# 3SAILab/two_stage_object_detection

Measured on AMD Instinct MI355X. Metric: images/sec Faster R-CNN ResNet-50 @800x1333, higher is better.
Workload: dtype f32 storage/accumulate; conv products as bf16x3 (3 exact bf16 pieces per operand, 6 bf16 MFMAs per product) in 0 of 43 conv layers, as fp16x2 (2 fp16 pieces of 2^e x per operand, 3 fp16 MFMAs per product; e follows the tensor's abs-max per forward: range words) in 43, f32 MFMA in the rest; 1 GPU; Full Faster R-CNN resnet50 inference forward, batch=1 per GPU, 3x800x1333, 80+1 classes, 3000->300 proposals; global_batch=1, parallelism=dp1, hip_graph=True, autotuned_tiles=True, steps_in_flight=4, tiles_tuned_on=this rank

## Files before the change

### include/tsod.h

```cpp
#ifndef TSOD_H
#define TSOD_H

#include <stddef.h>
#include <stdint.h>

#ifdef __cplusplus
extern "C" {
#endif

#define TSOD_VERSION 242

typedef void *tsod_stream_t;

typedef enum tsod_status {
    TSOD_OK = 0,
    TSOD_ERR_INVALID_ARG = -1,
    TSOD_ERR_UNSUPPORTED = -2,
    TSOD_ERR_ALIGNMENT = -3,
    TSOD_ERR_WORKSPACE = -4,
    TSOD_ERR_LAUNCH = -5
} tsod_status;

const char *tsod_status_str(int status);
int tsod_version(void);
// ... 1 lines not shown

enum { TSOD_ACT_NONE = 0, TSOD_ACT_PRELU = 1, TSOD_ACT_RELU6 = 2, TSOD_ACT_RELU = 3 };
enum { TSOD_TILE_AUTO = 0, TSOD_TILE_128x128 = 1, TSOD_TILE_128x64 = 2, TSOD_TILE_64x64 = 3, TSOD_TILE_64x128 = 4,
       TSOD_TILE_128x128_W8 = 5, TSOD_TILE_128x64_W8 = 6, TSOD_TILE_256x128_W8 = 7, TSOD_TILE_64x64_S1 = 8,
       TSOD_TILE_128x64_W8_S1 = 9, TSOD_TILE_64x64_S1_K64 = 10, TSOD_TILE_128x64_W8_S1_K64 = 11,
       TSOD_TILE_64x64_W1_S1 = 12, TSOD_TILE_128x64_W2_S1 = 13, TSOD_TILE_128x64_S1 = 14, TSOD_TILE_64x128_S1 = 15,
       TSOD_TILE_128x128_S1 = 16,
       TSOD_TILE_D128x128 = 17, TSOD_TILE_D64x128 = 18, TSOD_TILE_D256x128 = 19,
       TSOD_TILE_D64x128_S2 = 20 ,
       TSOD_TILE_D128x256 = 21 ,
       TSOD_TILE_D128x128_K32 = 22 ,
       TSOD_TILE_D192x128 = 23 ,
       TSOD_TILE_D64x128_K64 = 24 ,
       TSOD_TILE_COUNT = 25 };
enum { TSOD_PREC_F32 = 0, TSOD_PREC_BF16X3 = 1, TSOD_PREC_FP16X2 = 2 };
#define TSOD_MAX_SEGMENTS 16

typedef struct tsod_conv2d_desc {
    int32_t N, H, W;
    int32_t in_pitch;
    int32_t n_seg;
    int32_t seg_off[TSOD_MAX_SEGMENTS];
    int32_t seg_len[TSOD_MAX_SEGMENTS];
    int32_t Cout;
    int32_t out_pitch;
    int32_t out_off;
    int32_t KH, KW;
    int32_t stride;
    int32_t pad_h, pad_w;
    int32_t OH, OW;
// ... 17 lines not shown
int tsod_amax_reset(uint32_t *words, int32_t n_tensors, tsod_stream_t stream);
int tsod_absmax_f32(const float *x, int64_t n, uint32_t *amax_out, tsod_stream_t stream);

int tsod_host_mapped_pointer(void *host, void **device);
int tsod_word_publish_i32(const int32_t *src_device, int32_t *dst_mapped, tsod_stream_t stream);

int tsod_pack_conv_weight_f32(const float *w_oihw, int32_t Cout, int32_t Cin_src, int32_t KH, int32_t KW_src,
                              int32_t Cin, int32_t KW, float *w_packed, tsod_stream_t stream);

size_t tsod_conv_weight_bf16x3_bytes(int32_t Cout, int32_t K);
int tsod_pack_conv_weight_bf16x3(const float *w_packed , int32_t Cout, int32_t K, void *w_bf16x3,
                                 tsod_stream_t stream);
size_t tsod_conv_weight_fp16x2_bytes(int32_t Cout, int32_t K);
int tsod_pack_conv_weight_fp16x2(const float *w_packed , int32_t Cout, int32_t K, int32_t w_scale_exp,
                                 void *w_fp16x2, tsod_stream_t stream);

size_t tsod_conv2d_workspace_bytes(const tsod_conv2d_desc *d);
int tsod_conv2d_resolve(const tsod_conv2d_desc *d, int32_t *tile, int32_t *split_k);

int tsod_conv2d_f32(const tsod_conv2d_desc *d, const float *in, const float *w_packed,
                    const float *scale , const float *shift ,
                    const float *residual , float *out,
                    void *workspace, size_t workspace_bytes, tsod_stream_t stream);

int tsod_conv2d_dual_f32(const tsod_conv2d_desc *d, const float *in, const float *in2, const float *w_packed,
                         const float *scale, const float *shift, const float *residual, float *out,
                         void *workspace, size_t workspace_bytes, tsod_stream_t stream);

typedef struct tsod_bottleneck_desc {
    int32_t N, H, W;
// ... 404 lines not shown
```

### two_stage_object_detection_amd/_ffi.py

```python
from __future__ import annotations

import ctypes
import os
from ctypes import POINTER, Structure, byref, c_char_p, c_double, c_float, c_int, c_int32, c_int64, c_size_t, c_void_p
from typing import NamedTuple

import torch

_PKG_DIR = os.path.dirname(os.path.abspath(__file__))
LIB_PATH = os.environ.get("TSOD_LIB") or os.path.join(_PKG_DIR, "libtsod.so")

TSOD_MAX_SEGMENTS = 16
AMAX_WORDS, AMAX_STRIDE = 64, 64
AMAX_BYTES = AMAX_WORDS * AMAX_STRIDE
ACT_NONE, ACT_PRELU, ACT_RELU6, ACT_RELU = 0, 1, 2, 3
PREC_F32, PREC_BF16X3, PREC_FP16X2 = 0, 1, 2
PREC_NAMES = {0: "f32", 1: "bf16x3", 2: "fp16x2"}
TILE_AUTO, TILE_128x128, TILE_128x64, TILE_64x64, TILE_64x128 = 0, 1, 2, 3, 4


class Tile(NamedTuple):
    name: str
    rows: int
    precisions: tuple
# ... 27 lines not shown
    22: Tile("d128x128k32",    128, _SPLIT, dma=True),
    23: Tile("d192x128",       192, _FP16X2, dma=True),
    24: Tile("d64x128k64",     64,  _FP16X2, dma=True),
}


def tile_ids(precision: int) -> tuple:
    return tuple(t for t, row in TILES.items() if precision in row.precisions)


TILE_NAMES = {TILE_AUTO: "auto", **{t: row.name for t, row in TILES.items()}}
TILE_IDS = tile_ids(PREC_F32)
DMA_TILE_IDS = tuple(t for t, row in TILES.items() if row.dma)
BF16X3_TILE_IDS = tile_ids(PREC_BF16X3)
FP16X2_TILE_IDS = tile_ids(PREC_FP16X2)

class TsodError(RuntimeError):
    pass


class ConvDesc(Structure):
    _fields_ = [
        ("N", c_int32), ("H", c_int32), ("W", c_int32),
        ("in_pitch", c_int32), ("n_seg", c_int32),
        ("seg_off", c_int32 * TSOD_MAX_SEGMENTS), ("seg_len", c_int32 * TSOD_MAX_SEGMENTS),
        ("Cout", c_int32), ("out_pitch", c_int32), ("out_off", c_int32),
        ("KH", c_int32), ("KW", c_int32), ("stride", c_int32), ("pad_h", c_int32), ("pad_w", c_int32),
        ("OH", c_int32), ("OW", c_int32), ("act", c_int32), ("slope", c_float),
        ("res_pitch", c_int32), ("res_off", c_int32), ("tile", c_int32), ("split_k", c_int32), ("precision", c_int32),
        ("c2", c_int32), ("in2_pitch", c_int32), ("in2_off", c_int32), ("stride2", c_int32), ("H2", c_int32), ("W2", c_int32),
# ... 46 lines not shown


class GradNormResult(Structure):
    _fields_ = [("sum_sq", c_double), ("norm", c_float), ("coef", c_float)]


_SIGNATURES = {
    "tsod_status_str": (c_char_p, [c_int]),
    "tsod_version": (c_int, []),
    "tsod_device_cu_count": (c_int, []),
    "tsod_pack_conv_weight_f32": (c_int, [c_void_p, c_int32, c_int32, c_int32, c_int32, c_int32, c_int32, c_void_p, c_void_p]),
    "tsod_conv_weight_bf16x3_bytes": (c_size_t, [c_int32, c_int32]),
    "tsod_pack_conv_weight_bf16x3": (c_int, [c_void_p, c_int32, c_int32, c_void_p, c_void_p]),
    "tsod_conv_weight_fp16x2_bytes": (c_size_t, [c_int32, c_int32]),
    "tsod_pack_conv_weight_fp16x2": (c_int, [c_void_p, c_int32, c_int32, c_int32, c_void_p, c_void_p]),
    "tsod_conv2d_workspace_bytes": (c_size_t, [POINTER(ConvDesc)]),
    "tsod_conv2d_resolve": (c_int, [POINTER(ConvDesc), POINTER(c_int32), POINTER(c_int32)]),
    "tsod_conv2d_f32": (c_int, [POINTER(ConvDesc), c_void_p, c_void_p, c_void_p, c_void_p, c_void_p, c_void_p,
                                c_void_p, c_size_t, c_void_p]),
    "tsod_conv2d_dual_f32": (c_int, [POINTER(ConvDesc), c_void_p, c_void_p, c_void_p, c_void_p, c_void_p, c_void_p, c_void_p,
                                     c_void_p, c_size_t, c_void_p]),
    "tsod_bottleneck_wstream_bytes": (c_size_t, [c_int32, c_int32]),
    "tsod_bottleneck_proj_wstream_bytes": (c_size_t, [c_int32, c_int32]),
    "tsod_bottleneck_fp16x2": (c_int, [POINTER(BottleneckDesc), c_void_p, c_void_p, c_void_p, c_void_p, c_void_p]),
    "tsod_stem_wfrag_bytes": (c_size_t, []),
    "tsod_stem_fp16x2": (c_int, [POINTER(StemDesc), c_void_p, c_void_p, c_void_p, c_void_p, c_void_p]),
    "tsod_linear_f32": (c_int, [c_void_p, c_int32, c_int32, c_int32, c_void_p, c_void_p, c_int32, c_void_p, c_int32,
                                c_void_p, c_size_t, c_void_p]),
    "tsod_linear_workspace_bytes": (c_size_t, [c_int32, c_int32, c_int32]),
    "tsod_maxpool3x3s2_f32": (c_int, [c_void_p, c_int32, c_int32, c_int32, c_int32, c_int32, c_void_p, c_int32, c_void_p]),
# ... 295 lines not shown
```

### two_stage_object_detection_amd/csrc/conv_igemm_f32.hip

```cpp
#include "tsod_internal.h"
#include <array>
#include <limits.h>
#include <stdlib.h>

namespace {

typedef float f32x16 __attribute__((ext_vector_type(16)));
typedef __bf16 bf16x8 __attribute__((ext_vector_type(8)));
typedef _Float16 f16x8 __attribute__((ext_vector_type(8)));

constexpr int kPatchLD = 36;
constexpr int kChanTab = 512;

struct ConvParams {
    const float *in, *w, *scale, *shift, *res;
    float *out, *partial;
    int *tickets;
    unsigned part_bytes;
    int N, H, W, in_pitch;
    int n_seg, seg_off[TSOD_MAX_SEGMENTS], seg_end[TSOD_MAX_SEGMENTS];
    int Cin, Cout, out_pitch, out_off;
    int KH, KW, stride, pad_h, pad_w, OH, OW;
    int act;
    float slope;
// ... 1511 lines not shown
int validate(const tsod_conv2d_desc *d) {
    TSOD_REQUIRE(d != nullptr, TSOD_ERR_INVALID_ARG);
    TSOD_REQUIRE(d->N > 0 && d->H > 0 && d->W > 0 && d->Cout > 0 && d->KH > 0 && d->KW > 0, TSOD_ERR_INVALID_ARG);
    TSOD_REQUIRE(d->stride > 0 && d->pad_h >= 0 && d->pad_w >= 0 && d->OH > 0 && d->OW > 0, TSOD_ERR_INVALID_ARG);
    TSOD_REQUIRE(d->n_seg >= 1 && d->n_seg <= TSOD_MAX_SEGMENTS, TSOD_ERR_INVALID_ARG);
    TSOD_REQUIRE((d->in_pitch & 3) == 0 && d->in_pitch > 0, TSOD_ERR_ALIGNMENT);
    for (int s = 0; s < d->n_seg; ++s) {
        TSOD_REQUIRE(d->seg_len[s] > 0 && d->seg_off[s] >= 0, TSOD_ERR_INVALID_ARG);
        TSOD_REQUIRE((d->seg_len[s] & 3) == 0 && (d->seg_off[s] & 3) == 0, TSOD_ERR_ALIGNMENT);
        TSOD_REQUIRE(d->seg_off[s] + d->seg_len[s] <= d->in_pitch, TSOD_ERR_INVALID_ARG);
    }
    TSOD_REQUIRE(d->out_off >= 0 && d->out_pitch >= d->out_off + d->Cout, TSOD_ERR_INVALID_ARG);
    TSOD_REQUIRE((d->OH - 1) * d->stride - d->pad_h < d->H && (d->OW - 1) * d->stride - d->pad_w < d->W,
                 TSOD_ERR_INVALID_ARG);
    TSOD_REQUIRE(d->act >= TSOD_ACT_NONE && d->act <= TSOD_ACT_RELU, TSOD_ERR_INVALID_ARG);
    TSOD_REQUIRE(d->tile >= 0 && d->tile < TSOD_TILE_COUNT && d->split_k >= -2 && d->split_k <= 64, TSOD_ERR_INVALID_ARG);
    TSOD_REQUIRE(d->precision == TSOD_PREC_F32 || d->precision == TSOD_PREC_BF16X3 || d->precision == TSOD_PREC_FP16X2, TSOD_ERR_INVALID_ARG);
    TSOD_REQUIRE(d->tile == TSOD_TILE_AUTO || kTiles[d->tile].launch[d->precision], TSOD_ERR_UNSUPPORTED);
    if (d->precision == TSOD_PREC_FP16X2)
        TSOD_REQUIRE(d->a_scale_exp >= -24 && d->a_scale_exp <= 24 && d->w_scale_exp >= -40 && d->w_scale_exp <= 40, TSOD_ERR_INVALID_ARG);
    const int64_t M = (int64_t)d->N * d->OH * d->OW;
    TSOD_REQUIRE(M < (int64_t)INT_MAX, TSOD_ERR_UNSUPPORTED);
    if (d->c2 != 0) {
        TSOD_REQUIRE(d->c2 > 0 && (d->c2 & 3) == 0 && d->stride2 > 0 && d->H2 > 0 && d->W2 > 0, TSOD_ERR_INVALID_ARG);
        TSOD_REQUIRE((d->in2_pitch & 3) == 0 && (d->in2_off & 3) == 0, TSOD_ERR_ALIGNMENT);
        TSOD_REQUIRE(d->in2_off >= 0 && d->in2_off + d->c2 <= d->in2_pitch, TSOD_ERR_INVALID_ARG);
        TSOD_REQUIRE((d->OH - 1) * d->stride2 < d->H2 && (d->OW - 1) * d->stride2 < d->W2, TSOD_ERR_INVALID_ARG);
        TSOD_REQUIRE(d->n_seg == 1 && (d->KH * d->KW * d->seg_len[0]) % 32 == 0 && d->seg_len[0] % 32 == 0, TSOD_ERR_UNSUPPORTED);
    }
    return TSOD_OK;
}
// ... 152 lines not shown
    }
    return best;
}

uint64_t weight_image_bytes(int prec, int Cout, int K) {
    const uint64_t groups = (uint64_t)Cout * ((K + 7) / 8);
    return prec == TSOD_PREC_BF16X3 ? groups * 48 : prec == TSOD_PREC_FP16X2 ? groups * 32 : (uint64_t)Cout * K * sizeof(float);
}

}

extern "C" int tsod_conv2d_resolve(const tsod_conv2d_desc *d, int32_t *tile, int32_t *split_k) {
    const int rc = validate(d);
    if (rc != TSOD_OK) return rc;
    TSOD_REQUIRE(tile && split_k, TSOD_ERR_INVALID_ARG);
    const Sched s = resolve(d);
    TSOD_REQUIRE(s.cost < 1e299, TSOD_ERR_UNSUPPORTED);
    *tile = s.tile;
    *split_k = s.sk_q > 0 ? -2 : (s.rem_tiles == 0 ? 1 : (s.dp_tiles == 0 ? s.split : -1));
    return TSOD_OK;
}

extern "C" size_t tsod_conv2d_workspace_bytes(const tsod_conv2d_desc *d) {
    if (validate(d) != TSOD_OK) return 0;
    const Sched s = resolve(d);
    return s.cost < 1e299 ? s.ws_bytes : 0;
}

extern "C" int tsod_conv2d_f32(const tsod_conv2d_desc *d, const float *in, const float *w_packed, const float *scale,
                               const float *shift, const float *residual, float *out, void *workspace,
                               size_t workspace_bytes, tsod_stream_t stream) {
    if (d != nullptr && d->c2 != 0) return TSOD_ERR_INVALID_ARG;
    return tsod_conv2d_dual_f32(d, in, nullptr, w_packed, scale, shift, residual, out, workspace, workspace_bytes, stream);
}

extern "C" int tsod_conv2d_dual_f32(const tsod_conv2d_desc *d, const float *in, const float *in2, const float *w_packed,
                                    const float *scale, const float *shift, const float *residual, float *out,
                                    void *workspace, size_t workspace_bytes, tsod_stream_t stream) {
    const int rc = validate(d);
    if (rc != TSOD_OK) return rc;
    TSOD_REQUIRE(in && w_packed && out, TSOD_ERR_INVALID_ARG);
    TSOD_REQUIRE((d->c2 > 0) == (in2 != nullptr) && (!in2 || tsod_aligned16(in2)), TSOD_ERR_INVALID_ARG);
    TSOD_REQUIRE(tsod_aligned16(in) && tsod_aligned16(w_packed), TSOD_ERR_ALIGNMENT);
    if (residual) TSOD_REQUIRE(d->res_off >= 0 && d->res_pitch >= d->res_off + d->Cout, TSOD_ERR_INVALID_ARG);

    ConvParams p;
    p.in = in; p.w = w_packed; p.scale = scale; p.shift = shift; p.res = residual; p.out = out;
    p.N = d->N; p.H = d->H; p.W = d->W; p.in_pitch = d->in_pitch;
    p.n_seg = d->n_seg;
    int cum = 0;
    for (int s = 0; s < TSOD_MAX_SEGMENTS; ++s) {
        p.seg_off[s] = s < d->n_seg ? d->seg_off[s] : 0;
        if (s < d->n_seg) cum += d->seg_len[s];
        p.seg_end[s] = cum;
    }
    p.Cin = cum; p.Cout = d->Cout; p.out_pitch = d->out_pitch; p.out_off = d->out_off;
    p.KH = d->KH; p.KW = d->KW; p.stride = d->stride; p.pad_h = d->pad_h; p.pad_w = d->pad_w;
    p.OH = d->OH; p.OW = d->OW; p.act = d->act; p.slope = d->slope;
    p.res_pitch = d->res_pitch; p.res_off = d->res_off;
// ... 142 lines not shown
```

### two_stage_object_detection_amd/engine.py

```python
from __future__ import annotations

import math
from collections import OrderedDict
from ctypes import byref, c_int32
from typing import Callable, Sequence

import torch

from . import _ffi
from ._ffi import (ACT_NONE, ACT_PRELU, ACT_RELU, ACT_RELU6, TILE_NAMES, ConvDesc, TsodError, check, lib,
                   make_conv_desc, ptr, stream_ptr)


def fold_bn(bn: torch.nn.BatchNorm2d):
    var = bn.running_var.detach().double().cpu()
    mean = bn.running_mean.detach().double().cpu()
    gamma = bn.weight.detach().double().cpu() if bn.affine else torch.ones_like(var)
    beta = bn.bias.detach().double().cpu() if bn.affine else torch.zeros_like(var)
    scale = gamma / torch.sqrt(var + bn.eps)
    shift = beta - mean * scale
    return scale.float(), shift.float()


class PackedConv:
# ... 140 lines not shown
def fp16x2_activation_exp(absmax: float, headroom_bits: int = 4) -> int:
    if absmax == 0.0 or not math.isfinite(absmax):
        return 8
    return max(-24, min(8, int(math.floor(math.log2(65504.0 / (absmax * (1 << headroom_bits)))))))


def weights_fp16x2(pc):
    hit = getattr(pc, "w2", None)
    if hit is None:
        from . import hip_ops
        e = hip_ops.fp16x2_weight_scale_exp(pc.w)
        hit = pc.w2 = (_publish(hip_ops.pack_conv_weight_fp16x2(pc.w, e)), e)
    return hit


def prelu_slope(m: torch.nn.PReLU) -> float:
    if m.weight.numel() != 1:
        raise TsodError("only single-parameter nn.PReLU is supported (what the reference uses)")
    return float(m.weight.detach().cpu().item())


class BufferPool:

    def __init__(self, device):
        self.device = device
        self._free: dict[int, list[torch.Tensor]] = {}
        self.total_bytes = 0
        self.on_alloc = None

    def alloc(self, shape: Sequence[int], dtype=torch.float32) -> torch.Tensor:
# ... 21 lines not shown
        if out and out[-1][0] + out[-1][1] == off:
            out[-1] = (out[-1][0], out[-1][1] + ln)
        else:
            out.append((off, ln))
    return out


class ConvStep:
    __slots__ = ("desc", "args", "name", "flops", "ws_bytes", "pc", "fn", "plan", "x", "x2")
    W_ARG, WS_ARG = 3, 8

    def choose(self, tile: int, split_k: int, precision: int):
        d = self.desc
        d.tile, d.split_k, d.precision = int(tile), int(split_k), int(precision)
        if precision == _ffi.PREC_FP16X2:
            w2, e = weights_fp16x2(self.pc)
            d.a_scale_exp, d.w_scale_exp = int(self.plan.a_exps.get(self.name, FP16X2_A_SCALE_EXP)), int(e)
            d.range_flag = ptr(self.plan.range_flag)
            self.args[self.W_ARG] = ptr(w2)
        else:
            self.args[self.W_ARG] = ptr(weights_bf16x3(self.pc)) if precision == _ffi.PREC_BF16X3 else ptr(self.pc.w)

    def args_on(self, ws: torch.Tensor) -> list:
        a = list(self.args)
        a[self.WS_ARG], a[self.WS_ARG + 1] = ptr(ws), ws.numel()
        return a


class Plan:
    def __init__(self, device, packed: dict | None = None, *, range_flag=None, a_exps: dict | None = None, slot: int = 0,
                 on_calibrated=None, precision: int = 0):
# ... 293 lines not shown
            d = st.desc
            K = d.KH * d.KW * sum(d.seg_len[i] for i in range(d.n_seg)) + max(0, int(d.c2))
            ksteps = (K + 31) // 32
            M = d.N * d.OH * d.OW
            self._refresh_amax_for(st)
            cands = []
            for prec in (precisions if precisions is not None else (int(d.precision),)):
                for tile in _ffi.tile_ids(prec):
                    for split in (splits or (1, -1, -2, 2, 3, 4, 6, 8, 12, 16, 24, 32)):
                        if split > 1 and ksteps // split < 2:
                            continue
                        st.choose(tile, split, prec)
                        if lib().tsod_conv2d_workspace_bytes(byref(d)) > big.numel():
                            continue
                        cands.append((tile, split, prec))
            def time_candidate(tile, split, prec, n_reps):
                st.choose(tile, split, prec)
                args = st.args_on(big)
                s = stream_ptr()
                conv_fn = st.fn
                rc = conv_fn(*args, s)
                if rc != 0:
                    return None
                e0, e1 = torch.cuda.Event(enable_timing=True), torch.cuda.Event(enable_timing=True)
                if concurrent == 1:
                    e0.record()
                    for _ in range(n_reps):
                        rc |= conv_fn(*args, s)
                    e1.record()
                else:
# ... 36 lines not shown
                raise TsodError(f"autotune: no runnable (tile, split) candidate for {st.name}")
            def beyond_l2(tile, split, prec):
                st.choose(tile, split, prec)
                slabs = max(0, int(lib().tsod_conv2d_workspace_bytes(byref(d))) - (256 << 10))
                wbytes = d.Cout * K * (6 if prec == _ffi.PREC_BF16X3 else 4)
                tiles_m = -(-M // _ffi.TILES[tile].rows)
                return 2 * slabs + wbytes * (tiles_m if split == -2 else 8)
            close = [c for c in second_look if c[0] <= best[0] * 1.02]
            if len(close) > 1:
                best = min(close, key=lambda c: (beyond_l2(c[1], c[2], c[3]), c[0]))
            st.choose(best[1], best[2], best[3])
            n_short = max(1, int(in_sequence), int(keep_shortlist))
            if n_short > 1:
                short, per = [], {}
                for c in timed:
                    if per.get((c[1], c[3]), 0) < 2:
                        short.append(c)
                        per[(c[1], c[3])] = per.get((c[1], c[3]), 0) + 1
                    if len(short) >= n_short:
                        break
                for pr in sorted({c[3] for c in timed}):
                    if all(c[3] != pr for c in short):
                        short.append(next(c for c in timed if c[3] == pr))
            else:
                short = list(timed[:1])
            shortlist.append([(tile, split, prec) for _, tile, split, prec in short])
            by = {}
            for t_, tile, split, prec in timed:
                by.setdefault(prec, (tile, split))
            best_by_prec.append(by)
            results.append((st.name, best[0], best[1], best[2], st.flops, best[3]))
            if verbose:
                print(f"  {st.name:34s} {TILE_NAMES[best[1]]:8s} split {best[2]:3d} {_ffi.PREC_NAMES[best[3]]:6s} {best[0] * 1e3:8.1f} us "
# ... 410 lines not shown
```

### two_stage_object_detection_amd/hip_ops.py

```python
from __future__ import annotations

import contextlib
import ctypes
import math
import threading
from ctypes import byref, c_int32

import torch
from torch.autograd.function import once_differentiable

from . import _ffi
from ._ffi import ACT_NONE, TsodError, check, lib, make_conv_desc, ptr, require_cuda, stream_ptr


class _Arena:

    def __init__(self, zero: bool = False):
        self._buf = {}
        self._retired = {}
        self._zero = zero

    def _key(self, device):
        owner = getattr(_OWNER_TLS, "owner", None)
        if owner is not None:
# ... 81 lines not shown
    return out


def fp16x2_weight_scale_exp(w_packed: torch.Tensor) -> int:
    m = float(w_packed.abs().max())
    return 0 if m == 0.0 or not math.isfinite(m) else max(-40, min(40, int(math.floor(math.log2(16384.0 / m)))))


def pack_conv_weight_fp16x2(w_packed: torch.Tensor, w_scale_exp: int) -> torch.Tensor:
    require_cuda(w_packed, "pack_conv_weight_fp16x2")
    w_packed = w_packed.contiguous()
    cout = w_packed.shape[0]
    K = w_packed.numel() // cout
    out = torch.empty(lib().tsod_conv_weight_fp16x2_bytes(cout, K), dtype=torch.uint8, device=w_packed.device)
    check(lib().tsod_pack_conv_weight_fp16x2(ptr(w_packed), cout, K, int(w_scale_exp), ptr(out), stream_ptr()), "pack_conv_weight_fp16x2")
    return out


_W3_CACHE: dict = {}


def _w3_for(w_packed: torch.Tensor) -> torch.Tensor:
    if w_packed.is_inference():
        return pack_conv_weight_bf16x3(w_packed)
    key = (w_packed.data_ptr(), tuple(w_packed.shape), w_packed._version)
    hit = _W3_CACHE.get(key)
    if hit is None:
        if len(_W3_CACHE) >= 64:
            _W3_CACHE.clear()
        base = w_packed._base if w_packed._base is not None else w_packed
# ... 18 lines not shown
        Cout, KH, KW, Cin = w_packed.shape
    segs = [(0, Cin)] if segs is None else segs
    assert sum(s[1] for s in segs) == Cin, "segments must add up to the packed Cin"
    OH = (H + 2 * pad - KH) // stride + 1
    OW = (W + 2 * pad - (KW if kw_logical is None else kw_logical)) // stride + 1
    if out is None:
        out = torch.empty((N, OH, OW, Cout), dtype=torch.float32, device=x.device)
    assert out.is_contiguous() and out.shape[:3] == (N, OH, OW)
    d = make_conv_desc(N=N, H=H, W=W, in_pitch=P, segs=segs, Cout=Cout, out_pitch=out.shape[3], out_off=out_off,
                       KH=KH, KW=KW, stride=stride, pad_h=pad, pad_w=pad, OH=OH, OW=OW, act=act, slope=slope,
                       res_pitch=0 if residual is None else residual.shape[-1], res_off=0, tile=tile, split_k=split_k,
                       precision=precision, src2=src2)
    if precision == _ffi.PREC_FP16X2:
        if w2 is None:
            w_scale_exp = fp16x2_weight_scale_exp(w_packed)
            w2 = pack_conv_weight_fp16x2(w_packed, w_scale_exp)
        d.a_scale_exp, d.w_scale_exp = int(a_scale_exp), int(w_scale_exp)
        d.range_flag = ptr(range_flag)
        d.amax_in, d.amax_in2 = _word_ptr(amax_in), _word_ptr(amax_in2)
    d.amax_out = _word_ptr(amax_out)
    ws_bytes = lib().tsod_conv2d_workspace_bytes(byref(d))
    ws = CONV_ARENA.get(x.device, ws_bytes) if ws_bytes else None
    w_arg = (w3 if w3 is not None else _w3_for(w_packed)) if precision == _ffi.PREC_BF16X3 else (w2 if precision == _ffi.PREC_FP16X2 else w_packed)
    check(lib().tsod_conv2d_dual_f32(byref(d), ptr(x), ptr(x2), ptr(w_arg), ptr(scale), ptr(shift), ptr(residual), ptr(out),
                                     ptr(ws), ws_bytes, stream_ptr()), "conv2d")
    return out


def pack_bottleneck_wstream(w1: torch.Tensor, w2: torch.Tensor, w3: torch.Tensor, projection: bool = False):
    dev = w1.device
    cin, cout = w1.shape[1], w3.shape[0]
# ... 1485 lines not shown
```

### two_stage_object_detection_amd/models/hardnet_grads.py

```python
from __future__ import annotations

import torch
from torch.autograd.function import once_differentiable

from .. import _ffi, hip_ops
from ..engine import bn_fold_grads, bnt_copy


def _conv33_weight(d, C):
    return d[:, :, :C].reshape(9, C).t().reshape(C, 1, 3, 3)


def pw_copy(rec):
    rc, y = rec["rc"], rec["y"]
    return dict(index=rec["index"], off=rec["off"], cout=rec["cout"], segs=rec["segs"], seg_real=rec["seg_real"],
                slices=rec["slices"], w=rc.w.view(rc.cout, -1).clone(), scale=rc.scale.clone(), bn=rec["bn"],
                y=None if y is None else y[..., rec["y_off"]:rec["y_off"] + rc.cout].clone(), bnt=bnt_copy(rec.get("bnt")))


def dw_copy(rec):
    return dict(rec, dw=tuple(t.clone() if isinstance(t, torch.Tensor) else t for t in rec["dw"]),
                x=None if rec["x"] is None else (rec["x"][0].clone(), rec["x"][1]), dw_bnt=bnt_copy(rec.get("dw_bnt")))


# ... 131 lines not shown
    if getattr(old, "w3", None) is not None:
        old.w3.copy_(hip_ops.pack_conv_weight_bf16x3(old.w))
    if getattr(old, "w2", None) is not None:
        img, e = old.w2
        top = float(old.w.abs().max()) * 2.0 ** e
        if not (2.0 ** 12 <= top < 2.0 ** 15):
            e = hip_ops.fp16x2_weight_scale_exp(old.w)
            for plan in owner._plans.values():
                for st in plan.conv_steps:
                    if getattr(st.pc, "pack", st.pc) is old and int(st.desc.precision) == _ffi.PREC_FP16X2:
                        st.desc.w_scale_exp = int(e)
                        plan.graph = None
            owner._bump_version()
        img.copy_(hip_ops.pack_conv_weight_fp16x2(old.w, e))
        old.w2 = (img, e)


def copy_pack(owner, old, new):
    for o, t in zip(old, new):
        if isinstance(o, torch.Tensor):
            o.copy_(t)


def refresh_packs(owner):
    start = owner.__dict__.get("_watch_from")
    if start is None:
        return
    seen = owner.__dict__.setdefault("_pack_versions", {})
    stale = {}
    for u in owner._units():
# ... 11 lines not shown
```

Measured before the change: 1172 images/s.

## Add activation-resident fp16x2 expand kernel for 1x1 convs with autotuned split codes

Adds a dedicated kernel for stride-1 1x1 fp16x2 convolutions. It loads a full row panel of the input (K up to 512) into LDS once as hi/lo fp16 pieces, then streams pre-swizzled weights for several 64-channel output slices over that resident panel, with fused scale, shift, residual, activation and amax epilogue. New negative split_k codes select the panel size and slice grouping, and these codes are added as candidates to the tile autotuner. The aim is to stop re-reading and re-splitting the activations for every output tile. The cost is a second packed weight copy per eligible layer and more autotune candidates.

```diff
diff --git a/include/tsod.h b/include/tsod.h
--- a/include/tsod.h
+++ b/include/tsod.h
@@ -39,6 +39,8 @@
        TSOD_TILE_D64x128_K64 = 24 ,
        TSOD_TILE_COUNT = 25 };
 enum { TSOD_PREC_F32 = 0, TSOD_PREC_BF16X3 = 1, TSOD_PREC_FP16X2 = 2 };
+#define TSOD_SPLIT_EXPAND (-3)
+#define TSOD_SPLIT_EXPAND_FORCED (-4)
 #define TSOD_MAX_SEGMENTS 16
 
 typedef struct tsod_conv2d_desc {
@@ -86,6 +88,9 @@
 size_t tsod_conv_weight_fp16x2_bytes(int32_t Cout, int32_t K);
 int tsod_pack_conv_weight_fp16x2(const float *w_packed , int32_t Cout, int32_t K, int32_t w_scale_exp,
                                  void *w_fp16x2, tsod_stream_t stream);
+size_t tsod_conv_weight_expand_fp16x2_bytes(int32_t Cout, int32_t K);
+int tsod_pack_conv_weight_expand_fp16x2(const float *w_packed , int32_t Cout, int32_t K, int32_t w_scale_exp,
+                                        void *wstream, tsod_stream_t stream);
 
 size_t tsod_conv2d_workspace_bytes(const tsod_conv2d_desc *d);
 int tsod_conv2d_resolve(const tsod_conv2d_desc *d, int32_t *tile, int32_t *split_k);
diff --git a/two_stage_object_detection_amd/_ffi.py b/two_stage_object_detection_amd/_ffi.py
--- a/two_stage_object_detection_amd/_ffi.py
+++ b/two_stage_object_detection_amd/_ffi.py
@@ -65,6 +65,18 @@
 DMA_TILE_IDS = tuple(t for t, row in TILES.items() if row.dma)
 BF16X3_TILE_IDS = tile_ids(PREC_BF16X3)
 FP16X2_TILE_IDS = tile_ids(PREC_FP16X2)
+TILE_64x128_S1 = 15
+SPLIT_EXPAND, SPLIT_EXPAND_FORCED = -3, -4
+EXPAND_SPLITS = tuple(range(SPLIT_EXPAND, SPLIT_EXPAND_FORCED - 10, -1))
+
+
+def expand_split(rows: int, groups: int) -> int:
+    return SPLIT_EXPAND_FORCED - ((rows // 128) + 2 * (int(groups).bit_length() - 1))
+
+
+def is_expand_split(split_k: int) -> bool:
+    return SPLIT_EXPAND_FORCED - 9 <= int(split_k) <= SPLIT_EXPAND
+
 
 class TsodError(RuntimeError):
     pass
@@ -141,6 +153,8 @@
     "tsod_pack_conv_weight_bf16x3": (c_int, [c_void_p, c_int32, c_int32, c_void_p, c_void_p]),
     "tsod_conv_weight_fp16x2_bytes": (c_size_t, [c_int32, c_int32]),
     "tsod_pack_conv_weight_fp16x2": (c_int, [c_void_p, c_int32, c_int32, c_int32, c_void_p, c_void_p]),
+    "tsod_conv_weight_expand_fp16x2_bytes": (c_size_t, [c_int32, c_int32]),
+    "tsod_pack_conv_weight_expand_fp16x2": (c_int, [c_void_p, c_int32, c_int32, c_int32, c_void_p, c_void_p]),
     "tsod_conv2d_workspace_bytes": (c_size_t, [POINTER(ConvDesc)]),
     "tsod_conv2d_resolve": (c_int, [POINTER(ConvDesc), POINTER(c_int32), POINTER(c_int32)]),
     "tsod_conv2d_f32": (c_int, [POINTER(ConvDesc), c_void_p, c_void_p, c_void_p, c_void_p, c_void_p, c_void_p,
diff --git a/two_stage_object_detection_amd/csrc/conv_expand.h b/two_stage_object_detection_amd/csrc/conv_expand.h
--- /dev/null
+++ b/two_stage_object_detection_amd/csrc/conv_expand.h
@@ -0,0 +1,68 @@
+#pragma once
+#include <stdint.h>
+#include "../../include/tsod.h"
+
+#if defined(__HIPCC__)
+#define TSOD_EXPAND_HD __host__ __device__
+#else
+#define TSOD_EXPAND_HD
+#endif
+
+constexpr int kExpandForcedLast = TSOD_SPLIT_EXPAND_FORCED - 9;
+static inline bool tsod_expand_split(int split_k) { return split_k <= TSOD_SPLIT_EXPAND && split_k >= kExpandForcedLast; }
+
+constexpr int kExpandPatchBytes = 32 * 144;
+constexpr int kExpandLdsMax = 160 * 1024;
+
+TSOD_EXPAND_HD static inline int tsod_expand_pitch(int K) { return 2 * K + 16; }
+TSOD_EXPAND_HD static inline int tsod_expand_lds_bytes(int R, int K) { return 2 * R * tsod_expand_pitch(K) + 4 * kExpandPatchBytes + 64; }
+
+TSOD_EXPAND_HD static inline int tsod_expand_pi(int j) { return 16 * ((j >> 2) & 1) + 4 * (j >> 3) + (j & 3); }
+TSOD_EXPAND_HD static inline int tsod_expand_pi_inv(int r) { return (((r >> 2) & 3) << 3) | ((r >> 4) << 2) | (r & 3); }
+TSOD_EXPAND_HD static inline size_t tsod_expand_stream_offset(int K, int n, int g) {
+    const int q = n >> 6, cb = (n >> 5) & 1, j = tsod_expand_pi_inv(n & 31);
+    const int s = g >> 2, c = (g >> 1) & 1, hh = g & 1;
+    return ((size_t)(q * (K / 32) + s) * 2 + cb) * 4096 + (size_t)(32 * hh + j) * 64 + c * 32;
+}
+
+static inline bool tsod_expand_shape_ok(const tsod_conv2d_desc *d) {
+    if (d->precision != TSOD_PREC_FP16X2 || d->KH != 1 || d->KW != 1 || d->stride != 1 || d->pad_h != 0 || d->pad_w != 0) return false;
+    if (d->n_seg != 1 || d->c2 > 0 || d->OH != d->H || d->OW != d->W) return false;
+    const int K = d->seg_len[0];
+    if (K % 32 != 0 || K < 64 || K > 512 || d->Cout <= 0 || d->Cout % 64 != 0) return false;
+    if ((d->seg_off[0] | d->out_pitch | d->out_off | d->res_pitch | d->res_off) & 3) return false;
+    return true;
+}
+
+struct tsod_expand_pick_t {
+    int R, G, groups;
+};
+
+static inline bool tsod_expand_pick(int64_t M, int K, int Cout, int cus, int split_k, tsod_expand_pick_t *out) {
+    const int slices = Cout / 64;
+    if (split_k != TSOD_SPLIT_EXPAND) {
+        const int code = TSOD_SPLIT_EXPAND_FORCED - split_k, R = 64 << (code & 1);
+        int groups = 1 << (code >> 1);
+        if (tsod_expand_lds_bytes(R, K) > kExpandLdsMax) return false;
+        if (groups > slices) groups = slices;
+        out->R = R; out->G = (slices + groups - 1) / groups; out->groups = (slices + out->G - 1) / out->G;
+        return true;
+    }
+    double best = 1e300;
+    for (int R = 64; R <= 128; R += 64) {
+        if (tsod_expand_lds_bytes(R, K) > kExpandLdsMax) continue;
+        const int64_t panels = (M + R - 1) / R;
+        for (int G = slices; G >= 1; --G) {
+            const int groups = (slices + G - 1) / G;
+            if ((slices + groups - 1) / groups != G) continue;
+            const int64_t per_cu = (panels * groups + cus - 1) / cus;
+            const double work = (double)R * K / 256.0 + (double)G * (R / 64) * (3.0 * K / 16.0 + 10.0);
+            const double cost = (double)per_cu * work;
+            if (cost < best) { best = cost; out->R = R; out->G = G; out->groups = groups; }
+        }
+    }
+    return best < 1e299;
+}
+
+int tsod_conv_expand_launch(const tsod_conv2d_desc *d, const float *in, const void *wstream, const float *scale, const float *shift,
+                            const float *residual, float *out, tsod_stream_t stream);
diff --git a/two_stage_object_detection_amd/csrc/conv_expand.hip b/two_stage_object_detection_amd/csrc/conv_expand.hip
--- /dev/null
+++ b/two_stage_object_detection_amd/csrc/conv_expand.hip
@@ -0,0 +1,333 @@
+#include "tsod_internal.h"
+#include "conv_expand.h"
+#include <limits.h>
+
+namespace {
+
+typedef float f32x16 __attribute__((ext_vector_type(16)));
+typedef unsigned int u32x4 __attribute__((ext_vector_type(4)));
+
+constexpr unsigned kOOB = 0xFFFFFFF0u;
+constexpr int W_STEP = 8192;
+constexpr int P_PITCH = 144, P_BYTES = kExpandPatchBytes;
+
+struct ExpandParams {
+    const float *in, *res, *scale, *shift;
+    float *out;
+    const unsigned char *wstream;
+    int M, K, slices, G, groups;
+    unsigned in_row, in_off, out_row, out_off, res_row, res_off;
+    unsigned in_bytes, out_bytes, res_bytes;
+    float neg_slope, act_hi;
+    float a_scale, acc_scale;
+    int w_scale_exp;
+    const unsigned *amax_in;
+    unsigned *amax_out;
+    int *range_flag;
+};
+
+__device__ __forceinline__ float4 bload4(__amdgpu_buffer_rsrc_t r, unsigned off) {
+    const u32x4 v = __builtin_amdgcn_raw_buffer_load_b128(r, off, 0, 0);
+    return make_float4(__uint_as_float(v.x), __uint_as_float(v.y), __uint_as_float(v.z), __uint_as_float(v.w));
+}
+__device__ __forceinline__ float act(float v, float neg_slope, float hi) { return fminf(fmaxf(v, 0.f) + neg_slope * fminf(v, 0.f), hi); }
+
+struct WFrag { u32x4 h[2], l[2]; };
+struct AFrag { u32x4 h, l; };
+
+template <int R, int RING>
+__global__ void __launch_bounds__(256, 2) conv_expand_kernel(const ExpandParams p) {
+    constexpr int NB = R / 64;
+    constexpr int SLOTS = RING ? RING : 3, AHEAD = SLOTS - 1;
+    extern __shared__ __align__(16) unsigned char lds[];
+    const int tid = threadIdx.x, lane = tid & 63, wave = tid >> 6;
+    const int j = lane & 31, hh = lane >> 5;
+    const int cb = wave & 1, pb0 = wave >> 1;
+    const int pitch = tsod_expand_pitch(p.K), plane = R * pitch, KS = p.K >> 5;
+    unsigned char *patch = lds + 2 * plane + wave * P_BYTES;
+    float *scr = reinterpret_cast<float *>(lds + 2 * plane + 4 * P_BYTES);
+
+    const int nwg = (int)gridDim.x, per = nwg >> 3, r8 = nwg & 7, xcd = (int)blockIdx.x & 7;
+    const int item = (xcd < r8 ? xcd * (per + 1) : r8 * (per + 1) + (xcd - r8) * per) + ((int)blockIdx.x >> 3);
+    const int panel = item / p.groups, grp = item - panel * p.groups;
+    const int m0 = panel * R, q_begin = grp * p.G, q_end = min(q_begin + p.G, p.slices);
+    const __amdgpu_buffer_rsrc_t rs_x = __builtin_amdgcn_make_buffer_rsrc((void *)p.in, (short)0, (int)p.in_bytes, 0x00020000);
+    const __amdgpu_buffer_rsrc_t rs_o = __builtin_amdgcn_make_buffer_rsrc((void *)p.out, (short)0, (int)p.out_bytes, 0x00020000);
+    const __amdgpu_buffer_rsrc_t rs_r = __builtin_amdgcn_make_buffer_rsrc((void *)(p.res ? p.res : p.out), (short)0, (int)p.res_bytes, 0x00020000);
+
+    float a_scale = p.a_scale, acc_scale = p.acc_scale;
+    if (p.amax_in != nullptr) {
+        const int e = tsod_fp16x2_exp_from_bits(tsod_amax_reduce_bits(p.amax_in[lane * TSOD_AMAX_STRIDE_WORDS]));
+        a_scale = __uint_as_float((unsigned)(127 + e) << 23);
+        acc_scale = __uint_as_float((unsigned)(127 - e - p.w_scale_exp) << 23);
+    }
+    a_scale = __uint_as_float((unsigned)__builtin_amdgcn_readfirstlane((int)__float_as_uint(a_scale)));
+    acc_scale = __uint_as_float((unsigned)__builtin_amdgcn_readfirstlane((int)__float_as_uint(acc_scale)));
+
+    const int t_end = q_end * KS;
+    const u32x4 *wbase = reinterpret_cast<const u32x4 *>(p.wstream + cb * (W_STEP / 2) + lane * 64);
+    auto w_load = [&](int s, WFrag &f) {
+        if (s >= t_end) return;
+        const u32x4 *src = wbase + (size_t)s * (W_STEP / 16);
+        f.h[0] = src[0]; f.l[0] = src[1]; f.h[1] = src[2]; f.l[1] = src[3];
+    };
+    WFrag wf[SLOTS];
+    int t = q_begin * KS;
+#pragma unroll
+    for (int i = 0; i < AHEAD; ++i) w_load(t + i, wf[i]);
+    wf[AHEAD] = wf[0];
+
+    const int upr = p.K >> 2, n_it = (R * upr) >> 8;
+    const int drow = 256 / upr, dq = 256 - drow * upr;
+    int lrow = tid / upr, lq = tid - lrow * upr, srow = lrow, sq = lq;
+    auto advance = [&](int &row, int &q) {
+        row += drow; q += dq;
+        if (q >= upr) { q -= upr; ++row; }
+    };
+    auto x_load = [&](int it, float4 (&x)[4]) {
+#pragma unroll
+        for (int i = 0; i < 4; ++i) {
+            if (it + i >= n_it) break;
+            const int m = m0 + lrow;
+            x[i] = bload4(rs_x, m < p.M ? (unsigned)m * p.in_row + p.in_off + (unsigned)lq * 16u : kOOB);
+            advance(lrow, lq);
+        }
+    };
+    auto x_store = [&](int it, const float4 (&x)[4]) {
+#pragma unroll
+        for (int i = 0; i < 4; ++i) {
+            if (it + i >= n_it) break;
+            unsigned h0, l0, h1, l1;
+            tsod_split2_pair(x[i].x, x[i].y, a_scale, h0, l0);
+            tsod_split2_pair(x[i].z, x[i].w, a_scale, h1, l1);
+            unsigned char *dst = lds + srow * pitch + sq * 8;
+            *reinterpret_cast<uint2 *>(dst) = make_uint2(h0, h1);
+            *reinterpret_cast<uint2 *>(dst + plane) = make_uint2(l0, l1);
+            advance(srow, sq);
+        }
+    };
+    {
+        float4 xa[4], xb[4];
+        x_load(0, xa);
+        for (int it = 0; it < n_it; it += 8) {
+            x_load(it + 4, xb);
+            x_store(it, xa);
+            x_load(it + 8, xa);
+            x_store(it + 4, xb);
+        }
+    }
+
+    const int ep_px = lane >> 3, ep_q = lane & 7;
+    int afa[NB];
+    unsigned opix[NB][4], rpix[NB][4];
+#pragma unroll
+    for (int b = 0; b < NB; ++b) {
+        afa[b] = ((pb0 + 2 * b) * 32 + j) * pitch + hh * 16;
+#pragma unroll
+        for (int i = 0; i < 4; ++i) {
+            const int m = m0 + (pb0 + 2 * b) * 32 + ep_px + 8 * i;
+            const unsigned ch = (unsigned)(cb * 32 + ep_q * 4) * 4u;
+            opix[b][i] = m < p.M ? (unsigned)m * p.out_row + p.out_off + ch : kOOB;
+            rpix[b][i] = m < p.M ? (unsigned)m * p.res_row + p.res_off + ch : kOOB;
+        }
+    }
+    auto res_load = [&](int q, float4 (&r)[NB][4]) {
+        const unsigned chq = (unsigned)(q * 64) * 4u;
+#pragma unroll
+        for (int b = 0; b < NB; ++b)
+#pragma unroll
+            for (int i = 0; i < 4; ++i) r[b][i] = bload4(rs_r, (q < q_end && rpix[b][i] != kOOB) ? rpix[b][i] + chq : kOOB);
+    };
+    auto a_frags = [&](int off, AFrag (&f)[NB]) {
+#pragma unroll
+        for (int b = 0; b < NB; ++b) {
+            f[b].h = *reinterpret_cast<const u32x4 *>(lds + afa[b] + off);
+            f[b].l = *reinterpret_cast<const u32x4 *>(lds + afa[b] + off + plane);
+        }
+    };
+    float4 res_next[NB][4];
+    res_load(q_begin, res_next);
+    __syncthreads();
+
+    float amax = 0.f, chk = 0.f;
+    f32x16 acc[NB];
+    AFrag af[2][NB];
+    for (int q = q_begin; q < q_end; ++q) {
+        float4 res[NB][4];
+#pragma unroll
+        for (int b = 0; b < NB; ++b)
+#pragma unroll
+            for (int i = 0; i < 4; ++i) res[b][i] = res_next[b][i];
+        res_load(q + 1, res_next);
+#pragma unroll
+        for (int b = 0; b < NB; ++b)
+#pragma unroll
+            for (int e = 0; e < 16; ++e) acc[b][e] = 0.f;
+        a_frags(0, af[0]);
+        auto step = [&](int ks, const WFrag &w) {
+            a_frags(ks * 64 + 32, af[1]);
+#pragma unroll
+            for (int b = 0; b < NB; ++b) tsod_mfma3(acc[b], w.h[0], w.l[0], af[0][b].h, af[0][b].l);
+            if (ks + 1 < KS) a_frags(ks * 64 + 64, af[0]);
+#pragma unroll
+            for (int b = 0; b < NB; ++b) tsod_mfma3(acc[b], w.h[1], w.l[1], af[1][b].h, af[1][b].l);
+        };
+        if constexpr (RING == 0) {
+            for (int ks = 0; ks < KS; ++ks, ++t) {
+                w_load(t + 2, wf[2]);
+                step(ks, wf[0]);
+                wf[0] = wf[1];
+                wf[1] = wf[2];
+            }
+        } else {
+            for (int ks0 = 0; ks0 < KS; ks0 += RING) {
+#pragma unroll
+                for (int i = 0; i < RING; ++i, ++t) {
+                    w_load(t + AHEAD, wf[(i + AHEAD) % RING]);
+                    step(ks0 + i, wf[i]);
+                    __builtin_amdgcn_sched_barrier(0);
+                }
+            }
+        }
+        const unsigned chq = (unsigned)(q * 64) * 4u;
+        const int ch = q * 64 + cb * 32 + ep_q * 4;
+        float4 sv = make_float4(acc_scale, acc_scale, acc_scale, acc_scale), bv = make_float4(0.f, 0.f, 0.f, 0.f);
+        if (p.scale != nullptr) {
+            const float4 s4 = *reinterpret_cast<const float4 *>(p.scale + ch);
+            sv = make_float4(s4.x * acc_scale, s4.y * acc_scale, s4.z * acc_scale, s4.w * acc_scale);
+        }
+        if (p.shift != nullptr) bv = *reinterpret_cast<const float4 *>(p.shift + ch);
+#pragma unroll
+        for (int b = 0; b < NB; ++b) {
+#pragma unroll
+            for (int v = 0; v < 4; ++v) {
+                chk = fmaf(acc[b][4 * v], 0.f, fmaf(acc[b][4 * v + 1], 0.f, fmaf(acc[b][4 * v + 2], 0.f, fmaf(acc[b][4 * v + 3], 0.f, chk))));
+                *reinterpret_cast<float4 *>(patch + j * P_PITCH + (16 * hh + 4 * v) * 4) =
+                    make_float4(acc[b][4 * v], acc[b][4 * v + 1], acc[b][4 * v + 2], acc[b][4 * v + 3]);
+            }
+            asm volatile("s_waitcnt lgkmcnt(0)" ::: "memory");
+            float4 tt[4];
+#pragma unroll
+            for (int i = 0; i < 4; ++i) tt[i] = *reinterpret_cast<const float4 *>(patch + (ep_px + 8 * i) * P_PITCH + ep_q * 16);
+            asm volatile("s_waitcnt lgkmcnt(0)" ::: "memory");
+            float m4 = 0.f;
+#pragma unroll
+            for (int i = 0; i < 4; ++i) {
+                const float o0 = act(fmaf(tt[i].x, sv.x, bv.x + res[b][i].x), p.neg_slope, p.act_hi);
+                const float o1 = act(fmaf(tt[i].y, sv.y, bv.y + res[b][i].y), p.neg_slope, p.act_hi);
+                const float o2 = act(fmaf(tt[i].z, sv.z, bv.z + res[b][i].z), p.neg_slope, p.act_hi);
+                const float o3 = act(fmaf(tt[i].w, sv.w, bv.w + res[b][i].w), p.neg_slope, p.act_hi);
+                const float m = fmaxf(fmaxf(fabsf(o0), fabsf(o1)), fmaxf(fabsf(o2), fabsf(o3)));
+                m4 = fmaxf(m4, opix[b][i] != kOOB ? m : 0.f);
+                u32x4 o;
+                o.x = __float_as_uint(o0); o.y = __float_as_uint(o1); o.z = __float_as_uint(o2); o.w = __float_as_uint(o3);
+                __builtin_amdgcn_raw_buffer_store_b128(o, rs_o, opix[b][i] != kOOB ? opix[b][i] + chq : kOOB, 0, 0);
+            }
+            amax = fmaxf(amax, m4);
+        }
+    }
+    if (p.range_flag != nullptr && __any(!(chk == 0.f)) && lane == 0) atomicOr(p.range_flag, 1);
+    if (p.amax_out != nullptr) tsod_amax_commit(p.amax_out, amax, scr, tid, 256);
+}
+
+__global__ void __launch_bounds__(256)
+pack_weight_expand_kernel(const float *__restrict__ w, int Cout, int K, float scale, unsigned char *__restrict__ out) {
+    const int groups = K / 8;
+    const long total = (long)Cout * groups;
+    for (long t = (long)blockIdx.x * blockDim.x + threadIdx.x; t < total; t += (long)gridDim.x * blockDim.x) {
+        const int g = (int)(t % groups), n = (int)(t / groups);
+        u32x4 h, l;
+#pragma unroll
+        for (int e = 0; e < 4; ++e) {
+            const int k = g * 8 + 2 * e;
+            unsigned hv, lv;
+            tsod_split2_pair(w[(long)n * K + k], w[(long)n * K + k + 1], scale, hv, lv);
+            h[e] = hv;
+            l[e] = lv;
+        }
+        u32x4 *o = reinterpret_cast<u32x4 *>(out + tsod_expand_stream_offset(K, n, g));
+        o[0] = h;
+        o[1] = l;
+    }
+}
+
+int expand_cus() {
+    static const int cus = [] {
+        int dev = 0, n = 0;
+        if (hipGetDevice(&dev) == hipSuccess && hipDeviceGetAttribute(&n, hipDeviceAttributeMultiprocessorCount, dev) == hipSuccess && n > 0) return n;
+        (void)hipGetLastError();
+        return 256;
+    }();
+    return cus;
+}
+
+template <int R, int RING>
+bool expand_lds_ready() {
+    static const bool ok = hipFuncSetAttribute(reinterpret_cast<const void *>(conv_expand_kernel<R, RING>),
+                                               hipFuncAttributeMaxDynamicSharedMemorySize, kExpandLdsMax) == hipSuccess;
+    if (!ok) (void)hipGetLastError();
+    return ok;
+}
+
+}
+
+int tsod_conv_expand_launch(const tsod_conv2d_desc *d, const float *in, const void *wstream, const float *scale, const float *shift,
+                            const float *residual, float *out, tsod_stream_t stream) {
+    TSOD_REQUIRE(tsod_expand_shape_ok(d), TSOD_ERR_UNSUPPORTED);
+    TSOD_REQUIRE(tsod_aligned16(in) && tsod_aligned16(wstream) && tsod_aligned16(out) && (!residual || tsod_aligned16(residual)) &&
+                     (!scale || tsod_aligned16(scale)) && (!shift || tsod_aligned16(shift)), TSOD_ERR_ALIGNMENT);
+    TSOD_REQUIRE((reinterpret_cast<uintptr_t>(d->amax_in) & 63u) == 0 && (reinterpret_cast<uintptr_t>(d->amax_out) & 63u) == 0, TSOD_ERR_ALIGNMENT);
+    const int64_t M = (int64_t)d->N * d->H * d->W;
+    const int K = d->seg_len[0];
+    const uint64_t in_bytes = (uint64_t)M * d->in_pitch * 4, out_bytes = (uint64_t)M * d->out_pitch * 4;
+    const uint64_t res_bytes = residual ? (uint64_t)M * d->res_pitch * 4 : 0;
+    TSOD_REQUIRE(M < INT_MAX && in_bytes < 0xFFFFFFF0ull && out_bytes < 0xFFFFFFF0ull && res_bytes < 0xFFFFFFF0ull, TSOD_ERR_UNSUPPORTED);
+    tsod_expand_pick_t pick;
+    TSOD_REQUIRE(tsod_expand_pick(M, K, d->Cout, expand_cus(), d->split_k, &pick), TSOD_ERR_UNSUPPORTED);
+    ExpandParams p;
+    p.in = in; p.res = residual; p.scale = scale; p.shift = shift; p.out = out; p.wstream = static_cast<const unsigned char *>(wstream);
+    p.M = (int)M; p.K = K; p.slices = d->Cout / 64; p.G = pick.G; p.groups = pick.groups;
+    p.in_row = (unsigned)d->in_pitch * 4u; p.in_off = (unsigned)d->seg_off[0] * 4u;
+    p.out_row = (unsigned)d->out_pitch * 4u; p.out_off = (unsigned)d->out_off * 4u;
+    p.res_row = (unsigned)d->res_pitch * 4u; p.res_off = (unsigned)d->res_off * 4u;
+    p.in_bytes = (unsigned)in_bytes; p.out_bytes = (unsigned)out_bytes; p.res_bytes = (unsigned)res_bytes;
+    p.neg_slope = d->act == TSOD_ACT_NONE ? 1.f : (d->act == TSOD_ACT_PRELU ? d->slope : 0.f);
+    p.act_hi = d->act == TSOD_ACT_RELU6 ? 6.f : __builtin_huge_valf();
+    p.a_scale = ldexpf(1.f, d->a_scale_exp); p.acc_scale = ldexpf(1.f, -(d->a_scale_exp + d->w_scale_exp));
+    p.w_scale_exp = d->w_scale_exp;
+    p.amax_in = d->amax_in; p.amax_out = d->amax_out; p.range_flag = d->range_flag;
+    const int64_t grid = (M + pick.R - 1) / pick.R * pick.groups;
+    TSOD_REQUIRE(grid < 0x7FFFFFFF, TSOD_ERR_UNSUPPORTED);
+    const size_t lds = (size_t)tsod_expand_lds_bytes(pick.R, K);
+    const int ring = K % 256 == 0 ? 8 : (K % 128 == 0 ? 4 : 0);
+#define TSOD_EXPAND_LAUNCH(R_, RING_)                                                                                            \
+    do {                                                                                                                         \
+        TSOD_REQUIRE((expand_lds_ready<R_, RING_>()), TSOD_ERR_LAUNCH);                                                          \
+        hipLaunchKernelGGL((conv_expand_kernel<R_, RING_>), dim3((unsigned)grid), dim3(256), lds, tsod_stream(stream), p);       \
+    } while (0)
+    if (pick.R == 64) {
+        if (ring == 8) TSOD_EXPAND_LAUNCH(64, 8); else if (ring == 4) TSOD_EXPAND_LAUNCH(64, 4); else TSOD_EXPAND_LAUNCH(64, 0);
+    } else {
+        if (ring >= 4) TSOD_EXPAND_LAUNCH(128, 4); else TSOD_EXPAND_LAUNCH(128, 0);
+    }
+#undef TSOD_EXPAND_LAUNCH
+    return tsod_launch_status();
+}
+
+extern "C" size_t tsod_conv_weight_expand_fp16x2_bytes(int32_t Cout, int32_t K) {
+    if (Cout <= 0 || K <= 0 || Cout % 64 || K % 32) return 0;
+    return (size_t)(Cout / 64) * (K / 32) * W_STEP;
+}
+
+extern "C" int tsod_pack_conv_weight_expand_fp16x2(const float *w_packed, int32_t Cout, int32_t K, int32_t w_scale_exp, void *wstream,
+                                                   tsod_stream_t stream) {
+    TSOD_REQUIRE(w_packed && wstream, TSOD_ERR_INVALID_ARG);
+    TSOD_REQUIRE(Cout > 0 && K > 0 && w_scale_exp >= -40 && w_scale_exp <= 40, TSOD_ERR_INVALID_ARG);
+    TSOD_REQUIRE(Cout % 64 == 0 && K % 32 == 0, TSOD_ERR_UNSUPPORTED);
+    TSOD_REQUIRE(tsod_aligned16(wstream), TSOD_ERR_ALIGNMENT);
+    const long total = (long)Cout * (K / 8);
+    const int blocks = (int)(tsod_cdiv(total, 256) < 4096 ? tsod_cdiv(total, 256) : 4096);
+    hipLaunchKernelGGL(pack_weight_expand_kernel, dim3(blocks), dim3(256), 0, tsod_stream(stream), w_packed, Cout, K,
+                       ldexpf(1.f, w_scale_exp), static_cast<unsigned char *>(wstream));
+    return tsod_launch_status();
+}
diff --git a/two_stage_object_detection_amd/csrc/conv_igemm_f32.hip b/two_stage_object_detection_amd/csrc/conv_igemm_f32.hip
--- a/two_stage_object_detection_amd/csrc/conv_igemm_f32.hip
+++ b/two_stage_object_detection_amd/csrc/conv_igemm_f32.hip
@@ -2,6 +2,7 @@
 #include <array>
 #include <limits.h>
 #include <stdlib.h>
+#include "conv_expand.h"
 
 namespace {
 
@@ -1549,7 +1550,9 @@
     TSOD_REQUIRE((d->OH - 1) * d->stride - d->pad_h < d->H && (d->OW - 1) * d->stride - d->pad_w < d->W,
                  TSOD_ERR_INVALID_ARG);
     TSOD_REQUIRE(d->act >= TSOD_ACT_NONE && d->act <= TSOD_ACT_RELU, TSOD_ERR_INVALID_ARG);
-    TSOD_REQUIRE(d->tile >= 0 && d->tile < TSOD_TILE_COUNT && d->split_k >= -2 && d->split_k <= 64, TSOD_ERR_INVALID_ARG);
+    TSOD_REQUIRE(d->tile >= 0 && d->tile < TSOD_TILE_COUNT && d->split_k <= 64 &&
+                     (d->split_k >= -2 || (tsod_expand_split(d->split_k) && d->tile == TSOD_TILE_64x128_S1 && d->precision == TSOD_PREC_FP16X2)),
+                 TSOD_ERR_INVALID_ARG);
     TSOD_REQUIRE(d->precision == TSOD_PREC_F32 || d->precision == TSOD_PREC_BF16X3 || d->precision == TSOD_PREC_FP16X2, TSOD_ERR_INVALID_ARG);
     TSOD_REQUIRE(d->tile == TSOD_TILE_AUTO || kTiles[d->tile].launch[d->precision], TSOD_ERR_UNSUPPORTED);
     if (d->precision == TSOD_PREC_FP16X2)
@@ -1732,6 +1735,14 @@
     const int rc = validate(d);
     if (rc != TSOD_OK) return rc;
     TSOD_REQUIRE(tile && split_k, TSOD_ERR_INVALID_ARG);
+    if (tsod_expand_split(d->split_k)) {
+        tsod_expand_pick_t pick;
+        TSOD_REQUIRE(tsod_expand_shape_ok(d) && tsod_expand_pick((int64_t)d->N * d->H * d->W, d->seg_len[0], d->Cout, cu_count(), d->split_k, &pick),
+                     TSOD_ERR_UNSUPPORTED);
+        *tile = d->tile;
+        *split_k = d->split_k;
+        return TSOD_OK;
+    }
     const Sched s = resolve(d);
     TSOD_REQUIRE(s.cost < 1e299, TSOD_ERR_UNSUPPORTED);
     *tile = s.tile;
@@ -1740,7 +1751,7 @@
 }
 
 extern "C" size_t tsod_conv2d_workspace_bytes(const tsod_conv2d_desc *d) {
-    if (validate(d) != TSOD_OK) return 0;
+    if (validate(d) != TSOD_OK || tsod_expand_split(d->split_k)) return 0;
     const Sched s = resolve(d);
     return s.cost < 1e299 ? s.ws_bytes : 0;
 }
@@ -1761,6 +1772,8 @@
     TSOD_REQUIRE((d->c2 > 0) == (in2 != nullptr) && (!in2 || tsod_aligned16(in2)), TSOD_ERR_INVALID_ARG);
     TSOD_REQUIRE(tsod_aligned16(in) && tsod_aligned16(w_packed), TSOD_ERR_ALIGNMENT);
     if (residual) TSOD_REQUIRE(d->res_off >= 0 && d->res_pitch >= d->res_off + d->Cout, TSOD_ERR_INVALID_ARG);
+    if (tsod_expand_split(d->split_k))
+        return tsod_conv_expand_launch(d, in, w_packed, scale, shift, residual, out, stream);
 
     ConvParams p;
     p.in = in; p.w = w_packed; p.scale = scale; p.shift = shift; p.res = residual; p.out = out;
diff --git a/two_stage_object_detection_amd/engine.py b/two_stage_object_detection_amd/engine.py
--- a/two_stage_object_detection_amd/engine.py
+++ b/two_stage_object_detection_amd/engine.py
@@ -178,6 +178,22 @@
     return hit
 
 
+def weights_expand(pc):
+    hit = getattr(pc, "wx", None)
+    if hit is None:
+        from . import hip_ops
+        e = weights_fp16x2(pc)[1]
+        hit = pc.wx = (_publish(hip_ops.pack_conv_weight_expand_fp16x2(pc.w, e)), e)
+    return hit
+
+
+def expand_eligible(d) -> bool:
+    K = int(d.seg_len[0])
+    return (d.KH == 1 and d.KW == 1 and d.stride == 1 and d.pad_h == 0 and d.pad_w == 0 and d.n_seg == 1 and d.c2 <= 0 and
+            K % 32 == 0 and 64 <= K <= 512 and d.Cout % 64 == 0 and
+            (d.seg_off[0] | d.out_pitch | d.out_off | d.res_pitch | d.res_off) & 3 == 0)
+
+
 def prelu_slope(m: torch.nn.PReLU) -> float:
     if m.weight.numel() != 1:
         raise TsodError("only single-parameter nn.PReLU is supported (what the reference uses)")
@@ -229,7 +245,7 @@
         d = self.desc
         d.tile, d.split_k, d.precision = int(tile), int(split_k), int(precision)
         if precision == _ffi.PREC_FP16X2:
-            w2, e = weights_fp16x2(self.pc)
+            w2, e = weights_expand(self.pc) if _ffi.is_expand_split(split_k) else weights_fp16x2(self.pc)
             d.a_scale_exp, d.w_scale_exp = int(self.plan.a_exps.get(self.name, FP16X2_A_SCALE_EXP)), int(e)
             d.range_flag = ptr(self.plan.range_flag)
             self.args[self.W_ARG] = ptr(w2)
@@ -553,6 +569,8 @@
                         if lib().tsod_conv2d_workspace_bytes(byref(d)) > big.numel():
                             continue
                         cands.append((tile, split, prec))
+                if prec == _ffi.PREC_FP16X2 and splits is None and expand_eligible(d):
+                    cands.extend((_ffi.TILE_64x128_S1, split, prec) for split in _ffi.EXPAND_SPLITS)
             def time_candidate(tile, split, prec, n_reps):
                 st.choose(tile, split, prec)
                 args = st.args_on(big)
@@ -619,9 +637,10 @@
             if n_short > 1:
                 short, per = [], {}
                 for c in timed:
-                    if per.get((c[1], c[3]), 0) < 2:
+                    fam = (c[1], c[3], _ffi.is_expand_split(c[2]))
+                    if per.get(fam, 0) < 2:
                         short.append(c)
-                        per[(c[1], c[3])] = per.get((c[1], c[3]), 0) + 1
+                        per[fam] = per.get(fam, 0) + 1
                     if len(short) >= n_short:
                         break
                 for pr in sorted({c[3] for c in timed}):
diff --git a/two_stage_object_detection_amd/hip_ops.py b/two_stage_object_detection_amd/hip_ops.py
--- a/two_stage_object_detection_amd/hip_ops.py
+++ b/two_stage_object_detection_amd/hip_ops.py
@@ -119,6 +119,20 @@
     K = w_packed.numel() // cout
     out = torch.empty(lib().tsod_conv_weight_fp16x2_bytes(cout, K), dtype=torch.uint8, device=w_packed.device)
     check(lib().tsod_pack_conv_weight_fp16x2(ptr(w_packed), cout, K, int(w_scale_exp), ptr(out), stream_ptr()), "pack_conv_weight_fp16x2")
+    return out
+
+
+def pack_conv_weight_expand_fp16x2(w_packed: torch.Tensor, w_scale_exp: int) -> torch.Tensor:
+    require_cuda(w_packed, "pack_conv_weight_expand_fp16x2")
+    w_packed = w_packed.contiguous()
+    cout = w_packed.shape[0]
+    K = w_packed.numel() // cout
+    n = lib().tsod_conv_weight_expand_fp16x2_bytes(cout, K)
+    if n == 0:
+        raise _ffi.TsodError(f"pack_conv_weight_expand_fp16x2: Cout {cout} must be a multiple of 64 and K {K} of 32")
+    out = torch.empty(n, dtype=torch.uint8, device=w_packed.device)
+    check(lib().tsod_pack_conv_weight_expand_fp16x2(ptr(w_packed), cout, K, int(w_scale_exp), ptr(out), stream_ptr()),
+          "pack_conv_weight_expand_fp16x2")
     return out
 
 
@@ -167,7 +181,7 @@
     if precision == _ffi.PREC_FP16X2:
         if w2 is None:
             w_scale_exp = fp16x2_weight_scale_exp(w_packed)
-            w2 = pack_conv_weight_fp16x2(w_packed, w_scale_exp)
+            w2 = (pack_conv_weight_expand_fp16x2 if _ffi.is_expand_split(split_k) else pack_conv_weight_fp16x2)(w_packed, w_scale_exp)
         d.a_scale_exp, d.w_scale_exp = int(a_scale_exp), int(w_scale_exp)
         d.range_flag = ptr(range_flag)
         d.amax_in, d.amax_in2 = _word_ptr(amax_in), _word_ptr(amax_in2)
diff --git a/two_stage_object_detection_amd/models/hardnet_grads.py b/two_stage_object_detection_amd/models/hardnet_grads.py
--- a/two_stage_object_detection_amd/models/hardnet_grads.py
+++ b/two_stage_object_detection_amd/models/hardnet_grads.py
@@ -169,6 +169,9 @@
             owner._bump_version()
         img.copy_(hip_ops.pack_conv_weight_fp16x2(old.w, e))
         old.w2 = (img, e)
+        if getattr(old, "wx", None) is not None:
+            old.wx[0].copy_(hip_ops.pack_conv_weight_expand_fp16x2(old.w, e))
+            old.wx = (old.wx[0], e)
 
 
 def copy_pack(owner, old, new):
```

Result: no change. 1176 images/s (median of 5 runs) (+0.4%).
